# tmr4/T41_SDR

Hardware: AMD Instinct MI355X
Metric: MSamples/s I/Q through full RX chain, batch=4096; achieved HBM GB/s vs roofline (higher is better)
Workload: dtype f32; 1 GPU; configs[1]: batched SSB (USB 200-3000 Hz) RX chain, decimate-by-8 + 512-pt fast-conv + demod + interpolate-by-8, 4096 channels x 2048 complex f32 samples per frame per GPU, per-channel NCO, AGC off, 128 consecutive frames per channel per launch; batch=4096, frame_len=2048, fft_length=512, frames_per_launch=128, buffer_layout=channel-major, world_size_observed=1

## Files before the change

t41_sdr_amd/csrc/rx512_kernel.hpp:

```cpp
#pragma once
#include "rx_chains.hpp"

namespace t41 {

template <int PART, bool AGC = false>
struct Geo {
  static constexpr bool kResident = (PART == 0) && !AGC;
  static constexpr int kWaves = kResident ? 16 : 4;
  static constexpr int kTab = kResident ? 1024 : kLdsTabFloats;
  static constexpr int kTw1 = kResident ? 0 : kLdsTabTw1;
  static constexpr int kTw2 = kResident ? 448 : kLdsTabTw2;
  static constexpr int kSlice = kResident ? 2496 : kLdsFloatsPerWave;
  static constexpr int kTotal = kTab + kWaves * kSlice;
  static constexpr int kX = 0;
  static constexpr int kXF = kResident ? 1348 : kXFloats;
  static constexpr int kY1 = kXF;
  static constexpr int kOV = kY1 + kY1Floats;
  static constexpr int kH1 = kOV + 512;
  static constexpr int kScr = kResident ? 80 : 0;
  static constexpr int kI1 = kScr;
};
template <int MODE, int PART, bool AGC, bool PIPE>
using Rx512Geo = Geo<PART, geo4(MODE, AGC) && !PIPE>;
static_assert(!Geo<0>::kResident || Geo<0>::kTotal * sizeof(float) == 160 * 1024, "PART 0: one workgroup owns the CU's LDS");
// ... 3 lines not shown
              pipe_layout(7).second == pipe_layout(7).counters + ((size_t)7 + 16) * 32 * sizeof(float) && kPipeStatWords == 16,
              "rx512_kernel's pipe_err / pipe_stat / sam_slots arithmetic follows pipe_layout()");
static_assert(!Geo<0>::kResident || (Geo<0>::kH1 + 24 <= Geo<0>::kSlice && Geo<0>::kScr + 8 * kFftRow * 2 <= Geo<0>::kXF &&
                                     Geo<0>::kI1 + 284 <= Geo<0>::kXF && Geo<0>::kScr >= 68), "resident LDS layout");

constexpr int kPartMap = 4;
constexpr int kPartSet = 8;
constexpr int kPartA24 = 16;
constexpr int kPartOut = 32;
template <int MODE, bool DEBUG, int PARTM, bool PLAIN, bool AGC = false, bool WQ15 = false, bool SEGPAR = false, bool PIPE = false>
__global__ __launch_bounds__((Rx512Geo<MODE, (PARTM & 3), AGC, PIPE>::kWaves * 64), 4) void rx512_kernel(const RxArgs a) {
  T41RX_CLK_BEGIN();
  constexpr int PART = PARTM & 3;
  constexpr bool MAP = (PARTM & kPartMap) != 0;
  constexpr bool SET = (PARTM & kPartSet) != 0;
  constexpr bool A24 = (PARTM & kPartA24) != 0;
  constexpr bool OUT = (PARTM & kPartOut) != 0;
  static_assert(PART <= 2 && (PARTM & ~(3 | kPartMap | kPartSet | kPartA24 | kPartOut)) == 0,
                "PARTM = PART, PART + kPartMap, or PART + kPartMap + kPartSet, each of the mapped ones with or without kPartA24 and kPartOut");
  static_assert(!OUT || (MAP && PART == 0 && !DEBUG && !SEGPAR) || ((PARTM & ~kPartSet) == 2 + kPartOut && SEGPAR),
                "the output-map form is a twin of the mapped FFT_LENGTH 512 kernels without taps, and of the segment-parallel back kernel");
  static_assert(!A24 || (MAP && PART == 0 && !DEBUG && !SEGPAR), "the 24 kS/s form is a twin of the mapped FFT_LENGTH 512 kernels without taps");
  static_assert(!SET || (MAP && PART == 0 && !SEGPAR) || (PARTM == 2 + kPartOut + kPartSet && SEGPAR),
                "the set form is a twin of the mapped FFT_LENGTH 512 kernels, and of the back kernel's output-map form");
  static_assert(!MAP || PART != 2, "the back end of the long-FFT pipeline reads no antenna samples");
  static_assert(!SEGPAR || (PART == 1 && MODE != kModeNfm) || (PART == 2 && MODE == kModeSsb && !AGC), "SEGPAR variants");
  static_assert(!PIPE || ((AGC || MODE == kModeSam) && PART == 0 && !DEBUG && !SEGPAR),
                "PIPE: the pipelined variants -- AGC on (see agc_prep_pipe), the synchronous detector with the AGC off (sam_chain_pipe), or both (PSA)");
  constexpr bool PSAM = PIPE && MODE == kModeSam && !AGC;
  constexpr bool PSA = PIPE && MODE == kModeSam && AGC;
  constexpr int kPF = PSAM ? kPrefetchPipeSam : PIPE ? kPrefetchPipe : kPrefetch;
  typedef Rx512Geo<MODE, PART, AGC, PIPE> G;
  constexpr bool KEEP = G::kResident;
  constexpr int NW = G::kWaves;
  constexpr int kX = G::kX, kY1 = G::kY1, kScr = G::kScr, kI1 = G::kI1;
  __shared__ __attribute__((aligned(16))) float smem[G::kTotal];
  constexpr int L = 2048, D = 256, N = 512;
  const int seg = (PART == 0) ? 1 : a.seg;
  const size_t state_stride = state_floats(512 * seg);
  int lane = threadIdx.x & 63;
  const int wv = __builtin_amdgcn_readfirstlane(threadIdx.x >> 6);
  const int job = blockIdx.x * NW + wv;
  const int runs = SEGPAR ? (a.nframes + a.seg_run - 1) / a.seg_run : 1;
  const int ch = SEGPAR ? job / runs : job;
  const int seg0 = SEGPAR ? (job - ch * runs) * a.seg_run : 0;
  const int seg1 = SEGPAR ? (seg0 + a.seg_run < a.nframes ? seg0 + a.seg_run : a.nframes) : a.nframes;

  auto stage_tables = [&]() {
    const float4 *src = reinterpret_cast<const float4 *>(a.tab);
    float4 *dst = reinterpret_cast<float4 *>(smem);
    if (PART == 1) {
      if (threadIdx.x < 128) dst[threadIdx.x] = reinterpret_cast<const float4 *>(a.tab + kTabSinCos)[threadIdx.x];
    } else if (KEEP) {
      if (threadIdx.x < 224) dst[threadIdx.x] = src[kTabTw1 / 2 + threadIdx.x];
      else if (threadIdx.x >= 256 && threadIdx.x < 256 + 56)
        reinterpret_cast<float2 *>(smem)[G::kTw2 + threadIdx.x - 256] =
            a.tab[kTabTw2 + 64 * ((threadIdx.x - 256) >> 3) + ((threadIdx.x - 256) & 7)];
      else if (PIPE && threadIdx.x >= 320 && threadIdx.x < 332)
        reinterpret_cast<unsigned *>(smem)[kPipeFlags + threadIdx.x - 320] = 0u;
    } else if (MODE == kModeSam) {
      for (int i = threadIdx.x; i < 516; i += 256) smem[i] = reinterpret_cast<const float *>(a.tab + kTabSam)[i];
      for (int i = 512 / 2 + threadIdx.x; i < (512 + 448) / 2; i += 256) dst[i] = src[i];
      if (threadIdx.x < 56)
        reinterpret_cast<float2 *>(smem)[kLdsTabTw2 + threadIdx.x] = a.tab[kTabTw2 + 64 * (threadIdx.x >> 3) + (threadIdx.x & 7)];
    } else {
      for (int i = threadIdx.x; i < (512 + 448) / 2; i += 256) dst[i] = src[i];
// ... 11 lines not shown

  const cf *ltab = reinterpret_cast<const cf *>(smem);
  float *lds = smem + G::kTab + wv * G::kSlice;
  float *st = a.state + (size_t)ch * state_stride;
  typedef const __attribute__((address_space(4))) int *MapPtr;
  const int pset = SET ? ((MapPtr)a.set_of)[ch] : 0;
  const CoefPtr cf0 = SET ? (CoefPtr)a.coef + pset : (CoefPtr)a.coef;
  const NcoPtr nco = (NcoPtr)(a.nco + ch);
  const float2 *__restrict__ tab = a.tab;
  const float2 *__restrict__ ptab = SET ? a.tab + (size_t)pset * kTabEntries512 : a.tab;
  const auto chain_coef = [&]() {
    if constexpr (SET) return CoefBySet{a.coef, a.set_of + NW * (int)blockIdx.x};
    else return CoefOwn{cf0};
  }();
  typedef const __attribute__((address_space(4))) SetGains *GainPtr;
  SetGains sg{};
  if (SET) {
    const GainPtr gp = (GainPtr)a.set_gain + pset;
    sg.g_rf = gp->g_rf, sg.g_band = gp->g_band, sg.neg_iq_amp = gp->neg_iq_amp, sg.iq_phase = gp->iq_phase, sg.iq_corr_on = gp->iq_corr_on;
  }
  const int strm = MAP ? ((MapPtr)a.in_map)[ch] : ch;
  const int out_row = OUT ? ((MapPtr)a.out_map)[ch] : ch;
  const bool muted = OUT && out_row < 0;
  if (PART == 2 && muted) return;

  const NcoState *ncs_rd = reinterpret_cast<const NcoState *>(st + kStNco) + (PART == 0 ? 0 : a.nco_rd);
  NcoState *ncs = reinterpret_cast<NcoState *>(st + kStNco) + (PART == 0 ? 0 : (a.nco_rd ^ 1));
  const uint64_t raw_dphi = nco->phase_inc;
  const double raw_rs = nco->r_star_sq;
  const uint64_t raw_phase = ncs_rd->phase;
  const double raw_r = ncs_rd->r;
  const float raw_dc = st[kStMisc + kMiscDc];
  uint64_t dphi = 0, phase0 = 0;
  constexpr bool kKeepPl = KEEP && !AGC && MODE != kModeSam;
  uint64_t pl_keep = 0;
  double osc_r = 1.0;
  float dc_carry = 0.0f;
  bool transient = false;

  f2 dc2 = splat(0.0f);
  float4 pI0[2], pI1[2], pQ0[2], pQ1[2];
  float4 tailN = make_float4(0, 0, 0, 0);
  float2 tailNq = make_float2(0, 0);
  cf nfm_carry = splat(0.0f);
  float4 hist1c = make_float4(0, 0, 0, 0);
  float hist2c = 0.0f, audn[4] = {0.0f, 0.0f, 0.0f, 0.0f};
  float4 agrec = make_float4(0, 0, 0, 0);
  float2 agmag = make_float2(0, 0);
#ifdef T41RX_STAMP
  unsigned long long stamp_acc = 0, stamp_last;
  asm volatile("s_memtime %0\n\ts_waitcnt lgkmcnt(0)" : "=s"(stamp_last)::"memory");
  {
    unsigned hwid;
    asm volatile("s_getreg_b32 %0, hwreg(HW_REG_HW_ID)" : "=s"(hwid));
    unsigned xcc;
    asm volatile("s_getreg_b32 %0, hwreg(HW_REG_XCC_ID)" : "=s"(xcc));
    if (lane == 27) stamp_acc = hwid | ((unsigned long long)(xcc & 0xf) << 32);
    unsigned long long rt;
    asm volatile("s_memrealtime %0\n\ts_waitcnt lgkmcnt(0)" : "=s"(rt)::"memory");
    if (lane == 28) stamp_acc = rt;
  }
#endif
  auto x2_tail = [&](const float *end, float (&xp)[8]) {
    float wp[28];
#pragma unroll
    for (int i = 0; i < 7; ++i) {
      const float4 t = *reinterpret_cast<const float4 *>(end - 28 + 4 * i);
      wp[4 * i] = t.x;
      wp[4 * i + 1] = t.y;
      wp[4 * i + 2] = t.z;
      wp[4 * i + 3] = t.w;
    }
    f2 up[4];
#pragma unroll
    for (int u = 0; u < 4; ++u) up[u] = splat(0.0f);
#pragma unroll
    for (int b = 0; b < 24; b += 8) {
      float ci[16];
      load_taps<16>(ci, (CFloatPtr)cf0, kCoInt1 + 2 * b);
#pragma unroll
      for (int u = 0; u < 4; ++u) {
// ... 86 lines not shown
        } else {
          const LaneOff lof = fresh_off(4 * lane);
          pI0[1] = ldg_stream(gI - 256, lof);
          pQ0[1] = ldg_stream(gQ - 256, lof);
        }
      }
      float4 tailI;
      if (KEEP && carried) {
        tailI = WQ15 ? make_float4(q15_lo(tailNq.x), q15_hi(tailNq.x), q15_lo(tailNq.y), q15_hi(tailNq.y)) : tailN;
      } else if (!WQ15) {
        if (!carried) {
          const LaneOff lof = fresh_off(8 * lane);
          pI0[0] = ldg_stream(gI, lof);
          pI1[0] = ldg_stream(gI, lof, 4);
          pQ0[0] = ldg_stream(gQ, lof);
          pQ1[0] = ldg_stream(gQ, lof, 4);
        }
        tailI = ldg4(gI + (L - 256), fresh_off(4 * lane));
      } else {
        if (!carried) {
          const LaneOff lof = fresh_off(4 * lane);
          pI0[0] = ldg_stream(gI, lof);
          pQ0[0] = ldg_stream(gQ, lof);
        }
        const float2 t = *reinterpret_cast<const float2 *>(gI + (L - 256) / 2 + 2 * lane);
        tailI = make_float4(q15_lo(t.x), q15_hi(t.x), q15_lo(t.y), q15_hi(t.y));
      }
      float4 h1 = any_float4(), h2 = any_float4();
      float4 ovl0 = any_float4(), ovl1 = any_float4(), ovl2 = any_float4();
      if (!hist_carried && !preroll) {
        if (lane < 14) h1 = *reinterpret_cast<const float4 *>(st + kStDec1 + 4 * lane);
        if (lane < 24) h2 = *reinterpret_cast<const float4 *>(st + kStDec2 + 4 * lane);
        if (KEEP) {
          ovl0 = *reinterpret_cast<const float4 *>(st + kStOverlap + 4 * lane);
          ovl1 = *reinterpret_cast<const float4 *>(st + kStOverlap + 256 + 4 * lane);
          if (!A24 && !muted) {
            if (lane < 6) ovl2 = *reinterpret_cast<const float4 *>(st + kStInt1 + 4 * lane);
            if (lane < 8) hist2c = st[kStInt2 + lane];
          }
        }
      }
      float g_rf, g_rf_i, g_hp, g_hp_i, iq_phase_neg = 0.0f, iq_phase_pos = 0.0f;
      f2 g_iq = splat(1.0f);
      {
        const int iq_corr_on = SET ? sg.iq_corr_on : a.iq_corr_on;
        g_rf = SET ? sg.g_rf : a.g_rf;
        if (WQ15) g_rf *= 1.0f / 32768.0f;
        g_rf_i = (PLAIN && iq_corr_on) ? -g_rf : g_rf;
        g_hp = g_rf * (float)kHpB0;
        g_hp_i = (PLAIN && iq_corr_on) ? -g_hp : g_hp;
        if (!PLAIN) {
          const float gb = SET ? sg.g_band : a.g_band;
          const bool iq_on = iq_corr_on != 0;
          g_iq = f2{iq_on ? gb * (SET ? sg.neg_iq_amp : a.neg_iq_amp) : gb, gb};
          const float ph = iq_on ? (SET ? sg.iq_phase : a.iq_phase) : 0.0f;
          iq_phase_neg = ph < 0.0f ? ph : 0.0f;
          iq_phase_pos = ph > 0.0f ? ph : 0.0f;
        }
      }
      STAMP(16);
      if (first_iter) stage_tables();
      STAMP(17);
      if (preroll) {
      } else if (!WQ15) {
        if (!carried1) {
          const LaneOff lof = fresh_off(8 * lane);
          pI0[1] = ldg_stream(gI + 512, lof);
          pI1[1] = ldg_stream(gI + 512, lof, 4);
          pQ0[1] = ldg_stream(gQ + 512, lof);
          pQ1[1] = ldg_stream(gQ + 512, lof, 4);
        }
      } else if (!carried1) {
        const LaneOff lof = fresh_off(4 * lane);
        pI0[1] = ldg_stream(gI + 256, lof);
        pQ0[1] = ldg_stream(gQ + 256, lof);
      }

      wave_sync();
      if (!hist_carried && !preroll) {
        if (lane < 14) *reinterpret_cast<float4 *>(lds + kX + 2 * xpad(2 * lane)) = h1;
        if (lane < 24) *reinterpret_cast<float4 *>(lds + kY1 + y1slot(lane)) = h2;
        if (KEEP) {
          *reinterpret_cast<float4 *>(lds + G::kOV + 4 * lane) = ovl0;
          *reinterpret_cast<float4 *>(lds + G::kOV + 256 + 4 * lane) = ovl1;
          if (!A24 && !muted && lane < 6) *reinterpret_cast<float4 *>(lds + G::kH1 + 4 * lane) = ovl2;
        }
      }
      STAMP(18);
      if (first_iter) {
        dphi = uniform_u64(raw_dphi);
        if (kKeepPl) {
          unsigned n1 = (unsigned)(8 * lane + 1);
          asm volatile("" : "+v"(n1));
          pl_keep = (uint64_t)n1 * dphi;
        }
        phase0 = uniform_u64(raw_phase) + (uint64_t)f * (uint64_t)L * dphi;
        osc_r = uniform_f64(raw_r);
        dc_carry = uniform_f32(raw_dc);
        transient = !preroll && fabs(osc_r * osc_r - uniform_f64(raw_rs)) > 1e-13;
      }
      auto rebuild_from = [&](float4 rI0, float4 rI1, float4 rQ0, float4 rQ1, uint64_t phase_end) -> f2 {
        cf z[8];
        if (!WQ15) {
          z[0] = cf{rI0.x * g_hp_i, rQ0.x * g_hp};
          z[1] = cf{rI0.y * g_hp_i, rQ0.y * g_hp};
          z[2] = cf{rI0.z * g_hp_i, rQ0.z * g_hp};
          z[3] = cf{rI0.w * g_hp_i, rQ0.w * g_hp};
          z[4] = cf{rI1.x * g_hp_i, rQ1.x * g_hp};
          z[5] = cf{rI1.y * g_hp_i, rQ1.y * g_hp};
          z[6] = cf{rI1.z * g_hp_i, rQ1.z * g_hp};
          z[7] = cf{rI1.w * g_hp_i, rQ1.w * g_hp};
        } else {
          const float wi[4] = {rI0.x, rI0.y, rI0.z, rI0.w}, wq[4] = {rQ0.x, rQ0.y, rQ0.z, rQ0.w};
  #pragma unroll
          for (int k = 0; k < 4; ++k) {
            z[2 * k] = cf{q15_lo(wi[k]) * g_hp_i, q15_lo(wq[k]) * g_hp};
            z[2 * k + 1] = cf{q15_hi(wi[k]) * g_hp_i, q15_hi(wq[k]) * g_hp};
          }
        }
        f2 dcs = splat(0.0f);
        dc_highpass<8, !AGC && MODE != kModeSam>(z, dcs, lane, hp8.x, hp8.y);
        if (!PLAIN) {
  #pragma unroll
          for (int k = 0; k < 8; ++k) {
            z[k] *= g_iq;
            z[k].y = fmaf(iq_phase_neg, z[k].x, z[k].y);
            z[k].x = fmaf(iq_phase_pos, z[k].y, z[k].x);
          }
        }
        {
          const uint64_t P = phase_end - (uint64_t)(511 - 8 * lane) * dphi;
          const float2 t = reinterpret_cast<const float2 *>(smem)[(int)(P >> 56)];
          const uint32_t u = (uint32_t)(P >> 24);
          const float ang = (float)u * (float)(6.283185307179586476925 / 256.0 / 4294967296.0);
          const float a2 = ang * ang;
          const float sn = ang * fmaf(a2, -1.0f / 6.0f, 1.0f);
          const float cs = fmaf(a2, fmaf(a2, 1.0f / 24.0f, -0.5f), 1.0f);
          const cf base = cmul(cf{t.x, t.y}, cf{cs, sn});
  #pragma unroll
          for (int k = 0; k < 8; ++k) {
            const cf osc = cmul_s(base, cf{nco->wk[k][0], nco->wk[k][1]});
            z[k] = cmulc(z[k], osc);
          }
        }
        wave_sync();
        float *xw = lds + kX + 20 * lane;
  #pragma unroll
        for (int i = 0; i < 4; ++i)
          *reinterpret_cast<float4 *>(xw + 2 * (xpad(28 + 2 * i))) = make_float4(z[2 * i].x, z[2 * i].y, z[2 * i + 1].x, z[2 * i + 1].y);
        wave_sync();
        cf o1[2];
        auto pidx = [](int o) { return xpad(o); };
        fir_pair<kDec1Taps, 1, 5, 18, 6>(xw, pidx, cf0, kCoDec1, o1[0], o1[1]);
        float4 hh = any_float4();
// ... 3 lines not shown
        if (lane >= 40) *reinterpret_cast<float4 *>(lds + kY1 + y1slot(lane - 40)) = make_float4(o1[0].x, o1[0].y, o1[1].x, o1[1].y);
        wave_sync();
        return dcs;
      };
      f2 dc_pre = splat(0.0f);
      if (preroll) {
        const float4 rI0 = pI0[1], rI1 = WQ15 ? pI0[1] : pI1[1], rQ0 = pQ0[1], rQ1 = WQ15 ? pQ0[1] : pQ1[1];
        if (!WQ15) {
          const LaneOff lof = fresh_off(8 * lane);
          pI0[1] = ldg_stream(gI + 512, lof);
          pI1[1] = ldg_stream(gI + 512, lof, 4);
          pQ0[1] = ldg_stream(gQ + 512, lof);
          pQ1[1] = ldg_stream(gQ + 512, lof, 4);
        } else {
          const LaneOff lof = fresh_off(4 * lane);
          pI0[1] = ldg_stream(gI + 256, lof);
          pQ0[1] = ldg_stream(gQ + 256, lof);
        }
        dc_pre = rebuild_from(rI0, rI1, rQ0, rQ1, phase0);
        if ((f & (seg - 1)) == 0) dc_carry = uniform_f32(dc_pre.y);
      }

      if (PART == 0 || (f & (seg - 1)) == 0) {
        float4 tailF = tailI;
        if (PART != 0) {
          if (!WQ15) {
            tailF = ldg4(gI + (seg * L - 256), fresh_off(4 * lane));
          } else {
            const float2 t = *reinterpret_cast<const float2 *>(gI + (seg * L - 256) / 2 + 2 * lane);
            tailF = make_float4(q15_lo(t.x), q15_hi(t.x), q15_lo(t.y), q15_hi(t.y));
          }
        }
        const float x[4] = {tailF.x * g_rf, tailF.y * g_rf, tailF.z * g_rf, tailF.w * g_rf};
        dc2 = f2{(g_rf_i != g_rf) ? -dc_carry : dc_carry, dc_highpass_end_state<4, !AGC && MODE != kModeSam>(x, hp4.x, hp4.y)};
      } else if (preroll) {
        dc2 = dc_pre;
      }

      STAMP(15);
      cf y2[2][2];
      float2 osc_tab[4];
      uint32_t osc_u[4];
      {
        const uint64_t Pl = kKeepPl ? pl_keep : (uint64_t)(unsigned)(8 * lane + 1) * dphi;
  #pragma unroll
        for (int sb = 0; sb < 4; ++sb) {
          const uint64_t P = (phase0 + (uint64_t)(512 * sb) * dphi) + Pl;
          osc_u[sb] = (uint32_t)(P >> 24);
          osc_tab[sb] = (PART == 1) ? reinterpret_cast<const float2 *>(smem)[(int)(P >> 56)] : ldg2(tab + kTabSinCos, (unsigned)(P >> 56));
        }
      }

  #pragma unroll
      for (int rd = 0; rd < 2; ++rd) {
  #pragma unroll
        for (int h = 0; h < 2; ++h) {
          const int s = 2 * rd + h;
          cf z[8];
          if (!WQ15) {
            z[0] = cf{pI0[h].x * g_hp_i, pQ0[h].x * g_hp};
            z[1] = cf{pI0[h].y * g_hp_i, pQ0[h].y * g_hp};
            z[2] = cf{pI0[h].z * g_hp_i, pQ0[h].z * g_hp};
            z[3] = cf{pI0[h].w * g_hp_i, pQ0[h].w * g_hp};
            z[4] = cf{pI1[h].x * g_hp_i, pQ1[h].x * g_hp};
            z[5] = cf{pI1[h].y * g_hp_i, pQ1[h].y * g_hp};
            z[6] = cf{pI1[h].z * g_hp_i, pQ1[h].z * g_hp};
            z[7] = cf{pI1[h].w * g_hp_i, pQ1[h].w * g_hp};
// ... 23 lines not shown
            {
              static_assert(kTabEntries512 * 2 >= 2048 + 8, "the stand-in source of the last frame's prefetch covers a frame's offsets");
              const bool more = f + 1 < seg1;
              const float *nI = more ? gI + fstep : reinterpret_cast<const float *>(tab);
              const float *nQ = more ? gQ + fstep : reinterpret_cast<const float *>(tab);
              if (KEEP && s == 3) {
                if (!WQ15) {
                  tailN = ldg4(nI + (L - 256), fresh_off(4 * lane));
                } else {
                  tailNq = *reinterpret_cast<const float2 *>(nI + (L - 256) / 2 + 2 * lane);
                }
              }
              if (KEEP && kPF < 2 && s == 3) {
              } else if (!WQ15) {
                const int o = 512 * (s - 2);
                const LaneOff lof = fresh_off(8 * lane);
                pI0[h] = ldg_stream(nI + o, lof);
                pI1[h] = ldg_stream(nI + o, lof, 4);
                pQ0[h] = ldg_stream(nQ + o, lof);
                pQ1[h] = ldg_stream(nQ + o, lof, 4);
              } else {
                const int o = 256 * (s - 2);
                const LaneOff lof = fresh_off(4 * lane);
                pI0[h] = ldg_stream(nI + o, lof);
                pQ0[h] = ldg_stream(nQ + o, lof);
              }
            }
          } else if (s == 3 && !KEEP) {
            const cf *ov = reinterpret_cast<const cf *>(st + kStOverlap);
  #pragma unroll
            for (int j = 0; j < 4; ++j) v[j] = ov[64 * j + lane];
          }
          STAMP(s == 0 ? 14 : 0);
          dc_highpass<8, !AGC && MODE != kModeSam>(z, dc2, lane, hp8.x, hp8.y);
          if (!PLAIN) {
  #pragma unroll
            for (int k = 0; k < 8; ++k) {
              z[k] *= g_iq;
              z[k].y = fmaf(iq_phase_neg, z[k].x, z[k].y);
              z[k].x = fmaf(iq_phase_pos, z[k].y, z[k].x);
            }
          }
          STAMP(1);
          const int n0 = 512 * s + 8 * lane;
          if (DEBUG && a.dbg_pre && tap_row >= 0) {
            float *dp = a.dbg_pre + ((size_t)ch * tap_stride + tap_row) * (2 * L);
  #pragma unroll
            for (int k = 0; k < 8; ++k) {
              dp[n0 + k] = z[k].x;
              dp[L + n0 + k] = z[k].y;
            }
          }
          if (transient) {
            const NcoPtr nt = fresh_nco(nco);
            const double r_star_sq = uniform_f64(nt->r_star_sq);
            const double w_abs = uniform_f64(nt->w_abs);
            const double inv_r = 1.0 / sqrt(r_star_sq);
            double r = osc_r;
            float amp[8];
  #pragma unroll
            for (int k = 0; k < 8; ++k) amp[k] = 1.0f;
            for (int g = 0; g < 64; ++g) {
  #pragma unroll
              for (int k = 0; k < 8; ++k) {
                if (g == lane) amp[k] = (float)(r * inv_r);
                r = r * (1.95 - r * r) * w_abs;
              }
// ... 18 lines not shown
          for (int k = 0; k < 8; ++k) {
            const cf w = cf{ncw->wk[k][0], ncw->wk[k][1]};
            const cf osc = cmul_s(base, w);
            z[k] = cmulc(z[k], osc);
          }
          if (DEBUG && a.dbg_nco) {
            float *dn = a.dbg_nco + ((size_t)ch * a.nframes + f) * (2 * L);
  #pragma unroll
            for (int k = 0; k < 8; ++k) {
              dn[n0 + k] = z[k].x;
              dn[L + n0 + k] = z[k].y;
            }
          }
          STAMP(2);
          wave_sync();
          float *xw = lds + kX + 20 * lane;
  #pragma unroll
          for (int i = 0; i < 4; ++i)
            *reinterpret_cast<float4 *>(xw + 2 * (xpad(28 + 2 * i))) =
                make_float4(z[2 * i].x, z[2 * i].y, z[2 * i + 1].x, z[2 * i + 1].y);
          wave_sync();
          cf o1[2];
          {
            auto pidx = [](int o) { return xpad(o); };
            if (!AGC) fir_pair<kDec1Taps, 1, 5, 18, 6, 14>(xw, pidx, cf0, kCoDec1, o1[0], o1[1], z);
            else fir_pair<kDec1Taps, 1, 5, 18, 6>(xw, pidx, cf0, kCoDec1, o1[0], o1[1]);
          }
          STAMP(3);
          {
            float4 hh = any_float4();
            if (lane < 14) hh = lds4(lds + kX + 2 * xpad(512 + 2 * lane));
            wave_sync();
            if (lane < 14) *reinterpret_cast<float4 *>(lds + kX + 2 * xpad(2 * lane)) = hh;
            *reinterpret_cast<float4 *>(lds + kY1 + y1slot(24 + 64 * h + lane)) =
                make_float4(o1[0].x, o1[0].y, o1[1].x, o1[1].y);
          }
        }
        STAMP(4);
        if (rd == 1) {
          if (AGC) PRIO(1);
          else PRIO(2);
        }
        wave_sync();
        {
          auto planes = [](int o) { return y1slot(o >> 1) / 2; };
          fir_pair<kDec2Taps, 3, 5, 26, 6>(lds + kY1 + 4 * lane, planes, cf0, kCoDec2, y2[rd][0], y2[rd][1]);
        }
        STAMP(5);
      {
          float4 hh = any_float4();
          if (lane < 24) hh = lds4(lds + kY1 + y1slot(128 + lane));
          wave_sync();
          if (lane < 24) *reinterpret_cast<float4 *>(lds + kY1 + y1slot(lane)) = hh;
        }
      }
      phase0 += (uint64_t)L * dphi;
      if (PART == 0 || (f & (seg - 1)) == seg - 1) dc_carry = uniform_f32(dc2.y);

      STAMP(4);
      FRESH_LANE();
      wave_sync();
      if (SEGPAR && seg0 == 0 && f == seg1 - 1 && seg1 < a.nframes) {
        const size_t last = (size_t)(a.nframes - 1 - f) * L;
        float4 rI0, rI1, rQ0, rQ1;
        if (!WQ15) {
          const LaneOff lof = fresh_off(8 * lane);
          rI0 = ldg_stream(gI + last + 1536, lof);
          rI1 = ldg_stream(gI + last + 1536, lof, 4);
          rQ0 = ldg_stream(gQ + last + 1536, lof);
          rQ1 = ldg_stream(gQ + last + 1536, lof, 4);
        } else {
          const LaneOff lof = fresh_off(4 * lane);
          rI0 = rI1 = ldg_stream(gI + last / 2 + 768, lof);
          rQ0 = rQ1 = ldg_stream(gQ + last / 2 + 768, lof);
        }
        phase0 += (uint64_t)(a.nframes - 1 - f) * (uint64_t)L * dphi;
// ... 126 lines not shown
              }
            }
            au[rd][0] = (m0 < D - kDeemphTaps) ? acc.x : y2[rd][0].y;
            au[rd][1] = (m0 + 1 < D - kDeemphTaps) ? acc.y : y2[rd][1].y;
          }
          wave_sync();
        }
        if (PART == 0) {
          if (lane == 63) *reinterpret_cast<cf *>(st + kStMisc + kMiscNfmI) = y2[0][1];
        } else {
          if (lane == 63 && (f & (seg - 1)) == seg / 2 - 1) *reinterpret_cast<cf *>(st + kStMisc + kMiscNfmI) = y2[1][1];
          nfm_carry = cf{__int_as_float(__builtin_amdgcn_readlane(__float_as_int(y2[1][1].x), 63)),
                         __int_as_float(__builtin_amdgcn_readlane(__float_as_int(y2[1][1].y), 63))};
        }
  #pragma unroll
        for (int rd = 0; rd < 2; ++rd)
  #pragma unroll
          for (int e = 0; e < 2; ++e) y2[rd][e] = cf{au[rd][e], 0.0f};
      }
      if (PART == 1) {
        float *mid = a.mid + ((size_t)ch * a.nframes + f) * (2 * D);
  #pragma unroll
        for (int rd = 0; rd < 2; ++rd)
          *reinterpret_cast<float4 *>(mid + 2 * (128 * rd + 2 * lane)) =
              make_float4(y2[rd][0].x, y2[rd][0].y, y2[rd][1].x, y2[rd][1].y);
        continue;
      }


      {
        cf *tb = reinterpret_cast<cf *>(lds + kScr);
  #pragma unroll
        for (int rd = 0; rd < 2; ++rd)
          *reinterpret_cast<float4 *>(lds + kScr + 2 * (128 * rd + 2 * lane)) =
              make_float4(y2[rd][0].x, y2[rd][0].y, y2[rd][1].x, y2[rd][1].y);
        wave_sync();
  #pragma unroll
        for (int j = 0; j < 4; ++j) v[4 + j] = tb[lane + 64 * j];
        constexpr bool OVL_REAL = MODE == kModeNfm;
        if (KEEP) {
          cf *ov = reinterpret_cast<cf *>(lds + G::kOV);
  #pragma unroll
          for (int j = 0; j < 4; ++j) v[j] = ov[64 * j + lane];
  #pragma unroll
          for (int j = 0; j < 4; ++j) {
            if (OVL_REAL) ov[64 * j + lane].x = v[4 + j].x;
            else ov[64 * j + lane] = v[4 + j];
          }
        } else {
          cf *ov = reinterpret_cast<cf *>(st + kStOverlap);
  #pragma unroll
          for (int j = 0; j < 4; ++j) {
            if (OVL_REAL) ov[64 * j + lane].x = v[4 + j].x;
            else ov[64 * j + lane] = v[4 + j];
          }
        }
        if (OVL_REAL) {
  #pragma unroll
          for (int j = 0; j < 4; ++j) v[j].y = 0.0f;
        }
      }

      STAMP(6);
      FRESH_LANE();
      {
        cf tw1[7], tw2[7];
        cf mk[8];
        constexpr bool GMASK = KEEP || MODE == kModeSam;
        constexpr bool SMASK = SET && !GMASK;
        if (SMASK) {
  #pragma unroll
          for (int r = 0; r < 8; ++r) {
            const float2 t = ptab[kTabMask + 64 * r + lane];
// ... 463 lines not shown
      float c4[32];
      load_taps<32>(c4, (CFloatPtr)cf0, kCoInt2);
      const float x1[8] = {u1[0].x, u1[0].y, u1[1].x, u1[1].y, u1[2].x, u1[2].y, u1[3].x, u1[3].y};
#pragma unroll
      for (int i = 0; i < 7; ++i) {
        const float up = lane_up1(x1[i + 1]);
        const float hs = __int_as_float(__builtin_amdgcn_readlane(__float_as_int(hist2), i + 1));
        w[i] = write_lane<0>(up, hs);
      }
#pragma unroll
      for (int i = 0; i < 8; ++i) w[7 + i] = x1[i];
      if (!KEEP && lane == 63 && (!SEGPAR || (seg0 == 0 && seg1 == a.nframes))) {
        *reinterpret_cast<float4 *>(st + kStInt2) = make_float4(0.0f, x1[1], x1[2], x1[3]);
        *reinterpret_cast<float4 *>(st + kStInt2 + 4) = make_float4(x1[4], x1[5], x1[6], x1[7]);
      }
      if (PART == 2 && SEGPAR && seg0 == 0 && f == seg1 - 1 && seg1 < a.nframes) {
        const float *end = a.aud24 + ((size_t)ch * a.nframes + a.nframes) * D;
        if (lane < 6) *reinterpret_cast<float4 *>(st + kStInt1 + 4 * lane) = *reinterpret_cast<const float4 *>(end - 24 + 4 * lane);
        float xp[8];
        x2_tail(end, xp);
        if (lane == 0) {
          *reinterpret_cast<float4 *>(st + kStInt2) = make_float4(0.0f, xp[1], xp[2], xp[3]);
          *reinterpret_cast<float4 *>(st + kStInt2 + 4) = make_float4(xp[4], xp[5], xp[6], xp[7]);
        }
      }
      if (PART == 2 || KEEP) {
  #define T41RX_HIST2_ENTRY(i) hist2c = write_lane<i>(hist2c, __int_as_float(__builtin_amdgcn_readlane(__float_as_int(x1[i]), 63)));
        T41RX_HIST2_ENTRY(1) T41RX_HIST2_ENTRY(2) T41RX_HIST2_ENTRY(3) T41RX_HIST2_ENTRY(4) T41RX_HIST2_ENTRY(5) T41RX_HIST2_ENTRY(6) T41RX_HIST2_ENTRY(7)
  #undef T41RX_HIST2_ENTRY
      }
      wave_sync();
      unsigned qw[2] = {0u, 0u};
      constexpr bool PARK = KEEP && !WQ15;
      constexpr int kOvPark = (2048 - G::kOV + 3) / 4;
      static_assert(!PARK || (kOvPark > 0 && kOvPark <= 64 && G::kH1 >= 2048), "parking layout");
      float4 park_h = any_float4(), park_o = any_float4();
      if (PARK) {
        if (lane < 14) park_h = lds4(lds + kX + 2 * xpad(2 * lane));
        else if (lane >= 16 && lane < 40) park_h = lds4(lds + kY1 + y1slot(lane - 16));
        if (lane < kOvPark) park_o = lds4(lds + G::kOV + 4 * lane);
        wave_sync();
      }
      float *tr = PARK ? lds : lds + kScr;
#pragma unroll
      for (int u = 0; u < 8; ++u) {
        f2 o01 = splat(0.0f), o23 = splat(0.0f);
#pragma unroll
        for (int t = 0; t < 8; ++t) {
          const f2 x = splat(w[u + t]);
          o01 = pk_fma(x, f2{c4[4 * t + 3], c4[4 * t + 2]}, o01);
          o23 = pk_fma(x, f2{c4[4 * t + 1], c4[4 * t]}, o23);
        }
        if (!WQ15) {
          *reinterpret_cast<float4 *>(tr + 4 * (8 * lane + (u ^ (lane & 7)))) = make_float4(o01.x, o01.y, o23.x, o23.y);
        } else if ((u & 1) == 0) {
          qw[0] = q15_pack2(o01.x, o01.y);
          qw[1] = q15_pack2(o23.x, o23.y);
        } else {
          const int piece = u >> 1;
          *reinterpret_cast<uint4 *>(tr + 4 * (4 * lane + (piece ^ ((lane >> 1) & 3)))) =
              make_uint4(qw[0], qw[1], q15_pack2(o01.x, o01.y), q15_pack2(o23.x, o23.y));
        }
      }
      wave_sync();
      STAMP(12);
      if (!WQ15) {
        const LaneOff lof = fresh_off(4 * lane);
#pragma unroll
        for (int i = 0; i < 8; ++i) {
          const int row = 8 * i + (lane >> 3);
          const float4 t = lds4(tr + 4 * (8 * row + ((lane & 7) ^ (row & 7))));
          stg_stream(gO + 256 * i, lof, t);
        }
      } else {
        const LaneOff lof = fresh_off(4 * lane);
#pragma unroll
        for (int i = 0; i < 4; ++i) {
          const int row = 16 * i + (lane >> 2);
          const float4 t = lds4(tr + 4 * (4 * row + ((lane & 3) ^ ((row >> 1) & 3))));
          stg_stream(gO + 256 * i, lof, t);
        }
      }
      if (PARK) {
        wave_sync();
        if (lane < 14) *reinterpret_cast<float4 *>(lds + kX + 2 * xpad(2 * lane)) = park_h;
        else if (lane >= 16 && lane < 40) *reinterpret_cast<float4 *>(lds + kY1 + y1slot(lane - 16)) = park_h;
        if (lane < kOvPark) *reinterpret_cast<float4 *>(lds + G::kOV + 4 * lane) = park_o;
      }
    }
    STAMP(13);
#ifdef T41RX_PIPE_STAT
    if (PIPE && lane == 0)
      (reinterpret_cast<unsigned long long *>(a.agc_pipe + (size_t)a.nchan * kPipeSlots * kPipeSlotFloats) + (size_t)job * 16)[10] += __builtin_readcyclecounter() - ps_t;
#endif
  }
#ifdef T41RX_STAMP
  {
    unsigned long long rt;
    asm volatile("s_memrealtime %0\n\ts_waitcnt lgkmcnt(0)" : "=s"(rt)::"memory");
    if (lane == 29) stamp_acc = rt;
  }
  if (a.dbg_demod && PART != 2)
    reinterpret_cast<unsigned long long *>(a.dbg_demod + (size_t)a.nchan * a.nframes * D)[(size_t)ch * 64 + lane] = stamp_acc;
#endif

  if (PIPE && AGC && lane < 50) *reinterpret_cast<float4 *>(st + st_agc(512) + 4 * lane) = agrec;
  if (KEEP) {
    wave_sync();
    if (lane < 14) *reinterpret_cast<float4 *>(st + kStDec1 + 4 * lane) = lds4(lds + kX + 2 * xpad(2 * lane));
    if (lane < 24) *reinterpret_cast<float4 *>(st + kStDec2 + 4 * lane) = lds4(lds + kY1 + y1slot(lane));
    *reinterpret_cast<float4 *>(st + kStOverlap + 4 * lane) = lds4(lds + G::kOV + 4 * lane);
    *reinterpret_cast<float4 *>(st + kStOverlap + 256 + 4 * lane) = lds4(lds + G::kOV + 256 + 4 * lane);
    if (!A24 && !muted) {
      if (lane < 6) *reinterpret_cast<float4 *>(st + kStInt1 + 4 * lane) = lds4(lds + G::kH1 + 4 * lane);
      if (lane < 8) st[kStInt2 + lane] = (lane == 0) ? 0.0f : hist2c;
    }
  }
  if (PART != 2 && lane == 0) {
    if (!SEGPAR || seg0 == 0) {
      ncs->phase = phase0;
      ncs->r = osc_r;
      st[kStMisc + kMiscDc] = dc_carry;
    }
  }
  T41RX_CLK_END(job);
}

}
```

t41_sdr_amd/csrc/rx_device.hpp:

```cpp
#pragma once
#include <hip/hip_runtime.h>

#include <cstdlib>

#include "rx_experiments.hpp"
#include "rx_internal.hpp"
#include "rx_kernels.hpp"
#include "wave_fft.hpp"


namespace t41 {

constexpr int kPrefetch = 2;
constexpr int kPrefetchPipe = 0;
constexpr int kPrefetchPipeSam = 1;

#define PRIO(n) __builtin_amdgcn_s_setprio(n)
#define FRESH_LANE() asm volatile("" : "+v"(lane))
#define FRESH_WV(w) asm volatile("" : "+s"(w))

#ifdef T41RX_STAMP
#define STAMP(p)                                                                     \
  do {                                                                               \
    unsigned long long t_;                                                           \
// ... 159 lines not shown
  for (int k = 0; k < n; ++k) d = fmaf(a1, d, c * x[k]);
  const f2 B = hp_scan<n, FUSED>(f2{d, 0.0f}, m15, m31);
  return __int_as_float(__builtin_amdgcn_readlane(__float_as_int(B.x), 63));
}

template <int K>
__device__ __forceinline__ float write_lane(float old, float s) {
  asm("v_writelane_b32 %0, %1, %2" : "+v"(old) : "s"(s), "n"(K));
  return old;
}
__device__ __forceinline__ uint64_t uniform_u64(uint64_t v) {
  const uint32_t lo = __builtin_amdgcn_readfirstlane((uint32_t)v);
  const uint32_t hi = __builtin_amdgcn_readfirstlane((uint32_t)(v >> 32));
  return ((uint64_t)hi << 32) | lo;
}
__device__ __forceinline__ double uniform_f64(double v) {
  return __longlong_as_double((long long)uniform_u64((uint64_t)__double_as_longlong(v)));
}
__device__ __forceinline__ float uniform_f32(float v) {
  return __uint_as_float(__builtin_amdgcn_readfirstlane(__float_as_uint(v)));
}

constexpr int kLdsTabMask = 0, kLdsTabTw1 = 512, kLdsTabTw2 = 512 + 448;
constexpr int kLdsTabFloats = 2 * (512 + 448 + 56);
constexpr int kXFloats = 1352;
constexpr int kY1Floats = 608;
constexpr int kLdsFloatsPerWave = 2052;
static_assert(kXFloats + kY1Floats <= kLdsFloatsPerWave && kLdsFloatsPerWave >= 2048, "slice too small");
static_assert(kXFloats >= 8 * kFftRow * 2, "FFT exchange buffer must fit in X");
__device__ __forceinline__ constexpr int xpad(int j) { return j + ((j >> 3) << 1); }
constexpr int kY1Plane = 76;
__device__ __forceinline__ constexpr int y1slot(int s) { return 4 * ((s & 1) * kY1Plane + (s >> 1)); }

typedef const __attribute__((address_space(4))) DevCoef *CoefPtr;
__device__ __forceinline__ CoefPtr fresh_coef(CoefPtr p) {
  asm volatile("" : "+s"(p));
  return p;
}
struct CoefOwn {
  CoefPtr p;
  __device__ __forceinline__ CoefPtr of(int) const { return fresh_coef(p); }
};
struct CoefBySet {
  const DevCoef *base;
  const int *set_of;
  __device__ __forceinline__ const DevCoef *of(int c) const { return base + set_of[c]; }
};

__device__ __forceinline__ float4 lds4(const float *p) { return *reinterpret_cast<const float4 *>(p); }
__device__ __forceinline__ float4 any_float4() {
#pragma clang diagnostic push
#pragma clang diagnostic ignored "-Wuninitialized"
  float4 t;
  return t;
#pragma clang diagnostic pop
}
typedef float f4n __attribute__((ext_vector_type(4)));
__device__ __forceinline__ float4 ldg_stream(const float *p) {
  const f4n t = __builtin_nontemporal_load(reinterpret_cast<const f4n *>(p));
  return make_float4(t.x, t.y, t.z, t.w);
}
__device__ __forceinline__ void stg_stream(float *p, float4 v) {
  __builtin_nontemporal_store(f4n{v.x, v.y, v.z, v.w}, reinterpret_cast<f4n *>(p));
}
struct LaneOff {
  unsigned bytes;
// ... 85 lines not shown
}

__device__ __forceinline__ cf fir_mac(float tap, cf x, cf acc) {
  return pk_fma(splat(tap), x, acc);
}
template <int NT, int OFF0, int OFF1, int NLOAD, int GROUP, int TAIL0 = 1 << 20, typename IDX>
__device__ __forceinline__ void fir_pair(const float *win, IDX idx, CoefPtr coef, int taps, cf &acc0, cf &acc1,
                                         const cf *tail = nullptr) {
  constexpr int NTP = (NT + 7) & ~7;
  float tc[NTP];
  acc0 = splat(0.0f);
  acc1 = splat(0.0f);
#pragma unroll
  for (int l = 0; l < NLOAD; ++l) {
    if (l > 0 && (l % GROUP) == 0) asm volatile("" : "+v"(acc0), "+v"(acc1)::"memory");
    float4 t;
    if (tail && l >= TAIL0) t = make_float4(tail[2 * (l - TAIL0)].x, tail[2 * (l - TAIL0)].y, tail[2 * (l - TAIL0) + 1].x, tail[2 * (l - TAIL0) + 1].y);
    else t = lds4(win + 2 * idx(2 * l));
    const cf tv[2] = {cf{t.x, t.y}, cf{t.z, t.w}};
#pragma unroll
    for (int j = 0; j < 2; ++j) {
      const int x = 2 * l + j;
      const int i0 = x - OFF0, i1 = x - OFF1;
      if (i0 >= 0 && i0 < NT) {
        if ((i0 & 7) == 0) {
          float chunk[8];
          load_taps<8>(chunk, (CFloatPtr)coef, taps + i0);
#pragma unroll
          for (int q = 0; q < 8; ++q) tc[i0 + q] = chunk[q];
        }
        acc0 = fir_mac(tc[i0], tv[j], acc0);
      }
      if (i1 >= 0 && i1 < NT) acc1 = fir_mac(tc[i1], tv[j], acc1);
    }
  }
}

typedef const __attribute__((address_space(4))) ChanNco *NcoPtr;
__device__ __forceinline__ NcoPtr fresh_nco(NcoPtr p) {
  asm volatile("" : "+s"(p));
  return p;
}


#ifdef T41RX_CLK
static __device__ unsigned long long g_t41_clk[4 * 8192];
#define T41RX_CLK_BEGIN()                                                                                              \
  unsigned long long clk_c0, clk_r0;                                                                                   \
  asm volatile("s_memtime %0\n\ts_memrealtime %1\n\ts_waitcnt lgkmcnt(0)" : "=s"(clk_c0), "=s"(clk_r0)::"memory")
#define T41RX_CLK_END(wave_id)                                                                                         \
  do {                                                                                                                 \
    unsigned long long c1_, r1_;                                                                                       \
    unsigned hw_, xcc_;                                                                                                \
    asm volatile("s_waitcnt vmcnt(0)\n\ts_memtime %0\n\ts_memrealtime %1\n\ts_waitcnt lgkmcnt(0)" : "=s"(c1_), "=s"(r1_)::"memory"); \
    asm volatile("s_getreg_b32 %0, hwreg(HW_REG_HW_ID)" : "=s"(hw_));                                                  \
    asm volatile("s_getreg_b32 %0, hwreg(HW_REG_XCC_ID)" : "=s"(xcc_));                                                \
    if ((threadIdx.x & 63) == 0 && (wave_id) < 8192) {                                                                 \
      g_t41_clk[4 * (wave_id)] = c1_ - clk_c0;                                                                         \
      g_t41_clk[4 * (wave_id) + 1] = r1_ - clk_r0;                                                                     \
      g_t41_clk[4 * (wave_id) + 2] = clk_r0;                                                                           \
      g_t41_clk[4 * (wave_id) + 3] = hw_ | ((unsigned long long)(xcc_ & 0xf) << 32);                                   \
    }                                                                                                                  \
  } while (0)
#define T41RX_CLK_READER(name)                                                                                         \
  extern "C" __attribute__((visibility("default"))) int name(unsigned long long *host, int n) {                        \
    return (int)hipMemcpyFromSymbol(host, HIP_SYMBOL(g_t41_clk), sizeof(unsigned long long) * (size_t)n);              \
// ... 9 lines not shown
```

t41_sdr_amd/csrc/rx_experiments.hpp:

```cpp
#pragma once

#ifndef T41RX_EXPERIMENT
#define T41RX_EXPERIMENT 0
#endif
#if defined(T41RX_STAMP) || defined(T41RX_PIPE_STAT) || defined(T41RX_CLK)
#define T41RX_DIAGNOSTICS 1
#else
#define T41RX_DIAGNOSTICS 0
#endif
#if T41RX_DIAGNOSTICS && !T41RX_EXPERIMENT
#error "T41RX_STAMP / _PIPE_STAT / _CLK are diagnostic builds: pass -DT41RX_EXPERIMENT=1 with them (rx_experiments.hpp)"
#endif

namespace t41 {
constexpr int kKernelBuildFlags = T41RX_DIAGNOSTICS ? 2 : 0;
}

#define T41RX_BUILD_FLAGS(object) \
  int build_flags_##object() { return kKernelBuildFlags; }
```

Before: 412,400 MSamples/s.

## Keep SSB overlap block in registers and run decimate-by-2 FIR in one pass

For the resident SSB path, the 256-sample overlap-save block now stays in per-lane registers across frames instead of a round trip through LDS, and is loaded from and stored to global state only at the start and end. The second decimation stage switches to a four-plane Y1 layout with a multi-output FIR (fir_multi), producing all four outputs in a single pass after both rounds rather than one pair per round. The freed registers are traded by disabling the kept-phase and fused-scan paths only when the one-pass form is off. Extra register pressure could lower occupancy or cause spills, and the LDS layout changes affect parking and state save.

New measurement: 416,000 MSamples/s, median of 6. About the same (+0.9%).

```diff
diff --git a/t41_sdr_amd/csrc/rx512_kernel.hpp b/t41_sdr_amd/csrc/rx512_kernel.hpp
--- a/t41_sdr_amd/csrc/rx512_kernel.hpp
+++ b/t41_sdr_amd/csrc/rx512_kernel.hpp
@@ -59,6 +59,10 @@
   constexpr int kPF = PSAM ? kPrefetchPipeSam : PIPE ? kPrefetchPipe : kPrefetch;
   typedef Rx512Geo<MODE, PART, AGC, PIPE> G;
   constexpr bool KEEP = G::kResident;
+  constexpr bool OVREG = kFormOvReg && KEEP && MODE == kModeSsb && PLAIN && !AGC && !DEBUG && !WQ15;
+  constexpr bool ONEP = kFormDec2OnePass && OVREG;
+  static_assert(!ONEP || (kY1qFloats == kY1Floats + 512 && G::kH1 == G::kY1 + kY1qFloats), "ONEP: Y1 and the overlap block's slot, up to H1");
+  const auto ysl = [](int s) { return ONEP ? y1q(s) : y1slot(s); };
   constexpr int NW = G::kWaves;
   constexpr int kX = G::kX, kY1 = G::kY1, kScr = G::kScr, kI1 = G::kI1;
   __shared__ __attribute__((aligned(16))) float smem[G::kTotal];
@@ -136,7 +140,9 @@
   const double raw_r = ncs_rd->r;
   const float raw_dc = st[kStMisc + kMiscDc];
   uint64_t dphi = 0, phase0 = 0;
-  constexpr bool kKeepPl = KEEP && !AGC && MODE != kModeSam;
+  constexpr bool kRegsToSpare = !OVREG || ONEP;
+  constexpr bool kKeepPl = KEEP && !AGC && MODE != kModeSam && kRegsToSpare;
+  constexpr bool kScanFused = !AGC && MODE != kModeSam && kRegsToSpare;
   uint64_t pl_keep = 0;
   double osc_r = 1.0;
   float dc_carry = 0.0f;
@@ -151,6 +157,7 @@
   float hist2c = 0.0f, audn[4] = {0.0f, 0.0f, 0.0f, 0.0f};
   float4 agrec = make_float4(0, 0, 0, 0);
   float2 agmag = make_float2(0, 0);
+  cf ovp[4] = {splat(0.0f), splat(0.0f), splat(0.0f), splat(0.0f)};
 #ifdef T41RX_STAMP
   unsigned long long stamp_acc = 0, stamp_last;
   asm volatile("s_memtime %0\n\ts_waitcnt lgkmcnt(0)" : "=s"(stamp_last)::"memory");
@@ -303,8 +310,14 @@
         if (lane < 14) h1 = *reinterpret_cast<const float4 *>(st + kStDec1 + 4 * lane);
         if (lane < 24) h2 = *reinterpret_cast<const float4 *>(st + kStDec2 + 4 * lane);
         if (KEEP) {
-          ovl0 = *reinterpret_cast<const float4 *>(st + kStOverlap + 4 * lane);
-          ovl1 = *reinterpret_cast<const float4 *>(st + kStOverlap + 256 + 4 * lane);
+          if (OVREG) {
+            const cf *ov = reinterpret_cast<const cf *>(st + kStOverlap);
+  #pragma unroll
+            for (int j = 0; j < 4; ++j) ovp[j] = ov[64 * j + lane];
+          } else {
+            ovl0 = *reinterpret_cast<const float4 *>(st + kStOverlap + 4 * lane);
+            ovl1 = *reinterpret_cast<const float4 *>(st + kStOverlap + 256 + 4 * lane);
+          }
           if (!A24 && !muted) {
             if (lane < 6) ovl2 = *reinterpret_cast<const float4 *>(st + kStInt1 + 4 * lane);
             if (lane < 8) hist2c = st[kStInt2 + lane];
@@ -350,10 +363,12 @@
       wave_sync();
       if (!hist_carried && !preroll) {
         if (lane < 14) *reinterpret_cast<float4 *>(lds + kX + 2 * xpad(2 * lane)) = h1;
-        if (lane < 24) *reinterpret_cast<float4 *>(lds + kY1 + y1slot(lane)) = h2;
+        if (lane < 24) *reinterpret_cast<float4 *>(lds + kY1 + ysl(lane)) = h2;
         if (KEEP) {
-          *reinterpret_cast<float4 *>(lds + G::kOV + 4 * lane) = ovl0;
-          *reinterpret_cast<float4 *>(lds + G::kOV + 256 + 4 * lane) = ovl1;
+          if (!OVREG) {
+            *reinterpret_cast<float4 *>(lds + G::kOV + 4 * lane) = ovl0;
+            *reinterpret_cast<float4 *>(lds + G::kOV + 256 + 4 * lane) = ovl1;
+          }
           if (!A24 && !muted && lane < 6) *reinterpret_cast<float4 *>(lds + G::kH1 + 4 * lane) = ovl2;
         }
       }
@@ -390,7 +405,7 @@
           }
         }
         f2 dcs = splat(0.0f);
-        dc_highpass<8, !AGC && MODE != kModeSam>(z, dcs, lane, hp8.x, hp8.y);
+        dc_highpass<8, kScanFused>(z, dcs, lane, hp8.x, hp8.y);
         if (!PLAIN) {
   #pragma unroll
           for (int k = 0; k < 8; ++k) {
@@ -460,7 +475,7 @@
           }
         }
         const float x[4] = {tailF.x * g_rf, tailF.y * g_rf, tailF.z * g_rf, tailF.w * g_rf};
-        dc2 = f2{(g_rf_i != g_rf) ? -dc_carry : dc_carry, dc_highpass_end_state<4, !AGC && MODE != kModeSam>(x, hp4.x, hp4.y)};
+        dc2 = f2{(g_rf_i != g_rf) ? -dc_carry : dc_carry, dc_highpass_end_state<4, kScanFused>(x, hp4.x, hp4.y)};
       } else if (preroll) {
         dc2 = dc_pre;
       }
@@ -550,7 +565,7 @@
             for (int j = 0; j < 4; ++j) v[j] = ov[64 * j + lane];
           }
           STAMP(s == 0 ? 14 : 0);
-          dc_highpass<8, !AGC && MODE != kModeSam>(z, dc2, lane, hp8.x, hp8.y);
+          dc_highpass<8, kScanFused>(z, dc2, lane, hp8.x, hp8.y);
           if (!PLAIN) {
   #pragma unroll
             for (int k = 0; k < 8; ++k) {
@@ -635,7 +650,7 @@
             if (lane < 14) hh = lds4(lds + kX + 2 * xpad(512 + 2 * lane));
             wave_sync();
             if (lane < 14) *reinterpret_cast<float4 *>(lds + kX + 2 * xpad(2 * lane)) = hh;
-            *reinterpret_cast<float4 *>(lds + kY1 + y1slot(24 + 64 * h + lane)) =
+            *reinterpret_cast<float4 *>(lds + kY1 + (ONEP ? y1q(24 + 64 * s + lane) : y1slot(24 + 64 * h + lane))) =
                 make_float4(o1[0].x, o1[0].y, o1[1].x, o1[1].y);
           }
         }
@@ -645,6 +660,20 @@
           else PRIO(2);
         }
         wave_sync();
+        if (ONEP) {
+          if (rd == 1) {
+            cf yq[4];
+            auto planes = [](int o) { return y1q(o >> 1) / 2; };
+            fir_multi<kDec2Taps, 3, 2, 4, 1, 28, 6>(lds + kY1 + 4 * lane, planes, cf0, kCoDec2, yq);
+            y2[0][0] = yq[0], y2[0][1] = yq[1], y2[1][0] = yq[2], y2[1][1] = yq[3];
+            STAMP(5);
+            float4 hh = any_float4();
+            if (lane < 24) hh = lds4(lds + kY1 + y1q(256 + lane));
+            wave_sync();
+            if (lane < 24) *reinterpret_cast<float4 *>(lds + kY1 + y1q(lane)) = hh;
+          }
+          continue;
+        }
         {
           auto planes = [](int o) { return y1slot(o >> 1) / 2; };
           fir_pair<kDec2Taps, 3, 5, 26, 6>(lds + kY1 + 4 * lane, planes, cf0, kCoDec2, y2[rd][0], y2[rd][1]);
@@ -837,13 +866,20 @@
         cf *tb = reinterpret_cast<cf *>(lds + kScr);
   #pragma unroll
         for (int rd = 0; rd < 2; ++rd)
-          *reinterpret_cast<float4 *>(lds + kScr + 2 * (128 * rd + 2 * lane)) =
+          *reinterpret_cast<float4 *>(lds + kScr + 2 * (ONEP ? 4 * lane + 2 * rd : 128 * rd + 2 * lane)) =
               make_float4(y2[rd][0].x, y2[rd][0].y, y2[rd][1].x, y2[rd][1].y);
         wave_sync();
   #pragma unroll
         for (int j = 0; j < 4; ++j) v[4 + j] = tb[lane + 64 * j];
         constexpr bool OVL_REAL = MODE == kModeNfm;
-        if (KEEP) {
+        if (OVREG) {
+          static_assert(!OVREG || !OVL_REAL, "the real overlap-save writes half of the block: it keeps the LDS slot");
+  #pragma unroll
+          for (int j = 0; j < 4; ++j) {
+            v[j] = ovp[j];
+            ovp[j] = v[4 + j];
+          }
+        } else if (KEEP) {
           cf *ov = reinterpret_cast<cf *>(lds + G::kOV);
   #pragma unroll
           for (int j = 0; j < 4; ++j) v[j] = ov[64 * j + lane];
@@ -1373,13 +1409,13 @@
       wave_sync();
       unsigned qw[2] = {0u, 0u};
       constexpr bool PARK = KEEP && !WQ15;
-      constexpr int kOvPark = (2048 - G::kOV + 3) / 4;
-      static_assert(!PARK || (kOvPark > 0 && kOvPark <= 64 && G::kH1 >= 2048), "parking layout");
+      constexpr int kOvPark = OVREG ? 0 : (2048 - G::kOV + 3) / 4;
+      static_assert(!PARK || (((OVREG && kOvPark == 0) || (kOvPark > 0 && kOvPark <= 64)) && G::kH1 >= 2048), "parking layout");
       float4 park_h = any_float4(), park_o = any_float4();
       if (PARK) {
         if (lane < 14) park_h = lds4(lds + kX + 2 * xpad(2 * lane));
-        else if (lane >= 16 && lane < 40) park_h = lds4(lds + kY1 + y1slot(lane - 16));
-        if (lane < kOvPark) park_o = lds4(lds + G::kOV + 4 * lane);
+        else if (lane >= 16 && lane < 40) park_h = lds4(lds + kY1 + ysl(lane - 16));
+        if (kOvPark > 0 && lane < kOvPark) park_o = lds4(lds + G::kOV + 4 * lane);
         wave_sync();
       }
       float *tr = PARK ? lds : lds + kScr;
@@ -1425,8 +1461,8 @@
       if (PARK) {
         wave_sync();
         if (lane < 14) *reinterpret_cast<float4 *>(lds + kX + 2 * xpad(2 * lane)) = park_h;
-        else if (lane >= 16 && lane < 40) *reinterpret_cast<float4 *>(lds + kY1 + y1slot(lane - 16)) = park_h;
-        if (lane < kOvPark) *reinterpret_cast<float4 *>(lds + G::kOV + 4 * lane) = park_o;
+        else if (lane >= 16 && lane < 40) *reinterpret_cast<float4 *>(lds + kY1 + ysl(lane - 16)) = park_h;
+        if (kOvPark > 0 && lane < kOvPark) *reinterpret_cast<float4 *>(lds + G::kOV + 4 * lane) = park_o;
       }
     }
     STAMP(13);
@@ -1449,9 +1485,15 @@
   if (KEEP) {
     wave_sync();
     if (lane < 14) *reinterpret_cast<float4 *>(st + kStDec1 + 4 * lane) = lds4(lds + kX + 2 * xpad(2 * lane));
-    if (lane < 24) *reinterpret_cast<float4 *>(st + kStDec2 + 4 * lane) = lds4(lds + kY1 + y1slot(lane));
-    *reinterpret_cast<float4 *>(st + kStOverlap + 4 * lane) = lds4(lds + G::kOV + 4 * lane);
-    *reinterpret_cast<float4 *>(st + kStOverlap + 256 + 4 * lane) = lds4(lds + G::kOV + 256 + 4 * lane);
+    if (lane < 24) *reinterpret_cast<float4 *>(st + kStDec2 + 4 * lane) = lds4(lds + kY1 + ysl(lane));
+    if (OVREG) {
+      cf *ov = reinterpret_cast<cf *>(st + kStOverlap);
+#pragma unroll
+      for (int j = 0; j < 4; ++j) ov[64 * j + lane] = ovp[j];
+    } else {
+      *reinterpret_cast<float4 *>(st + kStOverlap + 4 * lane) = lds4(lds + G::kOV + 4 * lane);
+      *reinterpret_cast<float4 *>(st + kStOverlap + 256 + 4 * lane) = lds4(lds + G::kOV + 256 + 4 * lane);
+    }
     if (!A24 && !muted) {
       if (lane < 6) *reinterpret_cast<float4 *>(st + kStInt1 + 4 * lane) = lds4(lds + G::kH1 + 4 * lane);
       if (lane < 8) st[kStInt2 + lane] = (lane == 0) ? 0.0f : hist2c;
diff --git a/t41_sdr_amd/csrc/rx_device.hpp b/t41_sdr_amd/csrc/rx_device.hpp
--- a/t41_sdr_amd/csrc/rx_device.hpp
+++ b/t41_sdr_amd/csrc/rx_device.hpp
@@ -215,6 +215,10 @@
 constexpr int kY1Plane = 76;
 __device__ __forceinline__ constexpr int y1slot(int s) { return 4 * ((s & 1) * kY1Plane + (s >> 1)); }
 
+constexpr int kY1qPlane = 70;
+constexpr int kY1qFloats = 4 * 4 * kY1qPlane;
+__device__ __forceinline__ constexpr int y1q(int s) { return 4 * ((s & 3) * kY1qPlane + (s >> 2)); }
+
 typedef const __attribute__((address_space(4))) DevCoef *CoefPtr;
 __device__ __forceinline__ CoefPtr fresh_coef(CoefPtr p) {
   asm volatile("" : "+s"(p));
@@ -366,6 +370,39 @@
         acc0 = fir_mac(tc[i0], tv[j], acc0);
       }
       if (i1 >= 0 && i1 < NT) acc1 = fir_mac(tc[i1], tv[j], acc1);
+    }
+  }
+}
+
+template <int NT, int OFF0, int STEP, int NOUT, int L0, int NLOAD, int GROUP, typename IDX>
+__device__ __forceinline__ void fir_multi(const float *win, IDX idx, CoefPtr coef, int taps, cf (&acc)[NOUT]) {
+  constexpr int NTP = (NT + 7) & ~7;
+  float tc[NTP];
+#pragma unroll
+  for (int k = 0; k < NOUT; ++k) acc[k] = splat(0.0f);
+#pragma unroll
+  for (int l = L0; l < NLOAD; ++l) {
+    if (l > L0 && ((l - L0) % GROUP) == 0) {
+#pragma unroll
+      for (int k = 0; k < NOUT; ++k) asm volatile("" : "+v"(acc[k])::"memory");
+    }
+    const float4 t = lds4(win + 2 * idx(2 * l));
+    const cf tv[2] = {cf{t.x, t.y}, cf{t.z, t.w}};
+#pragma unroll
+    for (int j = 0; j < 2; ++j) {
+      const int x = 2 * l + j;
+#pragma unroll
+      for (int k = 0; k < NOUT; ++k) {
+        const int i = x - OFF0 - STEP * k;
+        if (i < 0 || i >= NT) continue;
+        if (k == 0 && (i & 7) == 0) {
+          float chunk[8];
+          load_taps<8>(chunk, (CFloatPtr)coef, taps + i);
+#pragma unroll
+          for (int q = 0; q < 8; ++q) tc[i + q] = chunk[q];
+        }
+        acc[k] = fir_mac(tc[i], tv[j], acc[k]);
+      }
     }
   }
 }
diff --git a/t41_sdr_amd/csrc/rx_experiments.hpp b/t41_sdr_amd/csrc/rx_experiments.hpp
--- a/t41_sdr_amd/csrc/rx_experiments.hpp
+++ b/t41_sdr_amd/csrc/rx_experiments.hpp
@@ -12,8 +12,19 @@
 #error "T41RX_STAMP / _PIPE_STAT / _CLK are diagnostic builds: pass -DT41RX_EXPERIMENT=1 with them (rx_experiments.hpp)"
 #endif
 
+#define T41RX_SW_PROBE_0 ~, 0,
+#define T41RX_SW_PROBE_1 ~, 1,
+#define T41RX_SW_PICK(a, b, ...) b
+#define T41RX_SW_TAKE(probe, dflt) T41RX_SW_PICK(probe dflt, dflt)
+#define T41RX_SW_GLUE(val, dflt) T41RX_SW_TAKE(T41RX_SW_PROBE_##val, dflt)
+#define T41RX_SWITCH(name, dflt) T41RX_SW_GLUE(name, dflt)
+
 namespace t41 {
-constexpr int kKernelBuildFlags = T41RX_DIAGNOSTICS ? 2 : 0;
+constexpr bool kFormOvReg = T41RX_SWITCH(T41RX_OV_REG, 1) != 0;
+constexpr bool kFormDec2OnePass = T41RX_SWITCH(T41RX_DEC2_ONEPASS, 1) != 0;
+constexpr bool kProductForm = kFormOvReg && kFormDec2OnePass;
+static_assert(kProductForm || T41RX_EXPERIMENT, "T41RX_OV_REG / _DEC2_ONEPASS other than the product's are experiment builds: pass -DT41RX_EXPERIMENT=1 with them (rx_experiments.hpp)");
+constexpr int kKernelBuildFlags = (T41RX_DIAGNOSTICS ? 2 : 0) | (kProductForm ? 0 : 4);
 }
 
 #define T41RX_BUILD_FLAGS(object) \
```
